# choice17/ransac_with_homography

Measured on AMD Instinct MI355X. Metric: backward-warp Mpixels/sec (+ RANSAC hypotheses/sec), higher is better.
Workload: dtype u8 (f64 coordinates, f32 blend); 1 GPU; transformImageH warp 3840x2160 RGB u8 bilinear -> 2028x3771 u8, 32 distinct frames per GPU per step, Hs mild perspective; full=False

## Files before the change

### ransac_with_homography_amd/csrc/rwh_warp_rgb8.h

```cpp
#pragma once
#include "rwh_common.h"
#include <type_traits>

namespace rwh {

typedef float f2 __attribute__((ext_vector_type(2)));

constexpr double MAGIC = 1572864.0;
constexpr uint32_t MAGIC_HI = 0x41380000u;
constexpr unsigned long long MAGIC_BITS = 0x4138000000000000ull;
constexpr float W_SCALE = 5.42101086242752217e-20f;
constexpr float U8_BIAS = -0.5f + 3.0517578125e-05f;

constexpr int FP_PX = 4;
constexpr int FP_ROWS = 9;
constexpr int FP_LANES = 21;
constexpr int FP_TEXELS = 4 * FP_LANES;
constexpr int FP_PITCH = 4 * FP_TEXELS + 16;

struct Coef {
    double cx[3], cy[3], cw[3];
    double dxs8[7][3];
    double ih[9];
    long long image;
// ... 838 lines not shown
            __builtin_amdgcn_wave_barrier();
            __builtin_amdgcn_fence(__ATOMIC_ACQUIRE, "wavefront");
        }
        const uint32_t bx = MAGIC_HI + (uint32_t)wxmn, by = MAGIC_HI + (uint32_t)wymn;
        const uint32_t rx_max = (uint32_t)(4 * wC - 2), ry_max = (uint32_t)(wnrows - 2);
#pragma unroll
        for (int h = 0; h < 2; ++h) {
            unsigned vbits = 0u;
            run_coords(h);
#pragma unroll
            for (int j = 0; j < FP_PX; ++j) {
                const bool valid = pixel_valid(j);
                weights2(lx[j], ly[j], valid ? WS : 0.f, valid ? WO : 0.f, valid ? WC : 0.f, wx0[j], wx1[j], wy0[j], wy1[j]);
                vbits |= (unsigned)valid << j;
                const uint32_t rx = min(hx[j] - bx, rx_max), ry = min(hy[j] - by, ry_max);
                const uint32_t lo = mad24_s(ry, (uint32_t)Win::LPITCH, rx << 2);
                const uint32_t* t0 = reinterpret_cast<const uint32_t*>(my + lo);
                const uint32_t* t1 = reinterpret_cast<const uint32_t*>(my + lo + Win::LPITCH);
                a0[j] = t0[0]; b0[j] = t0[1]; a1[j] = t1[0]; b1[j] = t1[1];
            }
            finish_masked_run(h, vbits);
        }
        return;
    }

    unsigned todo = 3u;
    if constexpr (HALVES) {
        todo = wpos ? 0u : 3u;
        if (wpos) {
            constexpr uint32_t lpitch = Win::LPITCH;
            chunk_t vh[2][Win::PASSES];
            int hrows[2];
            uint32_t tapc[2];
            bool hact[2];
#pragma unroll
            for (int h = 0; h < 2; ++h) {
                run_coords(h);
                const uint32_t lhx = h == 0 ? ehx[0] : hx[0], lhy = h == 0 ? ehy[0] : hy[0];
                const uint32_t rhx = h == 0 ? hx[3] : ehx[1], rhy = h == 0 ? hy[3] : ehy[1];
                const int hx0 = (int)__builtin_amdgcn_readlane(lhx, 0), hx1 = (int)__builtin_amdgcn_readlane(rhx, LPR - 1);
                const int hx2 = (int)__builtin_amdgcn_readlane(lhx, 64 - LPR), hx3 = (int)__builtin_amdgcn_readlane(rhx, 63);
                const int hy0 = (int)__builtin_amdgcn_readlane(lhy, 0), hy1 = (int)__builtin_amdgcn_readlane(rhy, LPR - 1);
                const int hy2 = (int)__builtin_amdgcn_readlane(lhy, 64 - LPR), hy3 = (int)__builtin_amdgcn_readlane(rhy, 63);
                const int qxmn = smin(smin(hx0, hx1), smin(hx2, hx3)) & ~3, qxmx = smax(smax(hx0, hx1), smax(hx2, hx3));
                const int qymn = smin(smin(hy0, hy1), smin(hy2, hy3)), qymx = smax(smax(hy0, hy1), smax(hy2, hy3));
                const int sxmn = (int)((uint32_t)smax(qxmn, 0) - MAGIC_HI), sxmx = (int)((uint32_t)smax(qxmx, 0) - MAGIC_HI);
                const int symn = (int)((uint32_t)smax(qymn, 0) - MAGIC_HI), symx = (int)((uint32_t)smax(qymx, 0) - MAGIC_HI);
                const int nr = symx - symn + 2, hC = (sxmx - sxmn + 5) >> 2;
                const bool hfits = (sxmn >= 0) & (sxmx < a.bound_w - 1) & (symn >= 0) & (symx < min(a.bound_h - 1, a.src_h - 2)) &
                                   (nr >= Win::RPP) & (nr <= Win::ROWS) & (hC <= Win::LPRW);
                hrows[h] = hfits ? nr : 0;
                hact[h] = (srow < Win::RPP) & (scol < hC);
                tapc[h] = ((uint32_t)qymn & 0xFFFFFFu) * lpitch + ((uint32_t)qxmn << 2) - slab_off_w;
                if (hfits) {
                    const unsigned char* gbase = simg + (size_t)((uint32_t)symn * pitch + (uint32_t)sxmn * (uint32_t)CH);
#pragma unroll
                    for (int p = 0; p < Win::PASSES; ++p)
                        if (p * Win::RPP < nr && hact[h])
                            __builtin_memcpy(&vh[h][p], gbase + (size_t)((uint32_t)min(p * Win::RPP, nr - Win::RPP) * pitch) + goff, sizeof(chunk_t));
                } else {
                    todo |= 1u << h;
                }
            }
#pragma unroll
            for (int h = 0; h < 2; ++h) {
                if (hrows[h] == 0) continue;
#pragma unroll
                for (int p = 0; p < Win::PASSES; ++p)
                    if (p * Win::RPP < hrows[h] && hact[h]) {
                        uint4 t4;
                        if constexpr (CH == 4) {
                            t4.x = vh[h][p].a; t4.y = vh[h][p].b; t4.z = vh[h][p].c; t4.w = vh[h][p].d;
                        } else {
                            t4.x = vh[h][p].a & 0xFFFFFFu;
                            t4.y = __builtin_amdgcn_perm(vh[h][p].b, vh[h][p].a, 0x0C050403u);
                            t4.z = __builtin_amdgcn_perm(vh[h][p].c, vh[h][p].b, 0x0C040302u);
                            t4.w = vh[h][p].c >> 8;
                        }
                        *reinterpret_cast<uint4*>(my + (uint32_t)min(p * Win::RPP, hrows[h] - Win::RPP) * lpitch + wl) = t4;
                    }
                __builtin_amdgcn_fence(__ATOMIC_RELEASE, "wavefront");
                __builtin_amdgcn_wave_barrier();
                __builtin_amdgcn_fence(__ATOMIC_ACQUIRE, "wavefront");
                if (h == 0) run_coords(0);
#pragma unroll
                for (int j = 0; j < FP_PX; ++j) {
                    weights2(lx[j], ly[j], WS, WO, WC, wx0[j], wx1[j], wy0[j], wy1[j]);
                    const uint32_t lo = mad24_s(hy[j], lpitch, shl2_add_s(hx[j], 0u - tapc[h]));
                    const uint32_t* t0 = reinterpret_cast<const uint32_t*>(slab0 + lo);
                    const uint32_t* t1 = reinterpret_cast<const uint32_t*>(slab0 + lo + lpitch);
                    a0[j] = t0[0]; b0[j] = t0[1]; a1[j] = t1[0]; b1[j] = t1[1];
                }
                const int first = tshift - (lcol + (PW / 2) * h);
                blend_store<DstT, PSTR, CH, true>(a0, b0, a1, b1, wx0, wx1, wy0, wy1, drow + CH * (PW / 2) * h,
                                                  store_any & (first <= 3 * PSTR), max(first, 0));
                __builtin_amdgcn_fence(__ATOMIC_RELEASE, "wavefront");
                __builtin_amdgcn_wave_barrier();
                if (h == 0 && hrows[1] != 0) run_coords(1);
            }
        }
        if (todo == 0u) return;
    }

#pragma unroll
    for (int h = 0; h < 2; ++h) {
        uint32_t off[FP_PX];
        bool near_end = false;
        unsigned vbits = 0u;
        if (HALVES && !(todo & (1u << h))) continue;
        run_coords(h);
#pragma unroll
        for (int j = 0; j < FP_PX; ++j) {
            const bool valid = pixel_valid(j);
            const int ix = (int)(hx[j] - MAGIC_HI), iy = (int)(hy[j] - MAGIC_HI);
            weights2(lx[j], ly[j], valid ? WS : 0.f, valid ? WO : 0.f, valid ? WC : 0.f, wx0[j], wx1[j], wy0[j], wy1[j]);
            off[j] = valid ? (uint32_t)iy * pitch + (uint32_t)ix * (uint32_t)CH : 0u;
            near_end |= valid & (iy > a.src_h - 3);
            vbits |= (unsigned)valid << j;
        }
        if (!__any(vbits != 0u)) {
#pragma unroll
            for (int j = 0; j < FP_PX; ++j) { a0[j] = 0u; b0[j] = 0u; a1[j] = 0u; b1[j] = 0u; }
        } else if (!__any(near_end)) {
#pragma unroll
            for (int j = 0; j < FP_PX; ++j) {
                const pk2 r0 = ld8(simg + off[j]);
                const pk2 r1 = ld8(simg + off[j] + pitch);
                if constexpr (CH == 4) { a0[j] = r0.a; b0[j] = r0.b; a1[j] = r1.a; b1[j] = r1.b; }
                else {
                    a0[j] = r0.a & 0xFFFFFFu; b0[j] = __builtin_amdgcn_perm(r0.b, r0.a, 0x0C050403u);
                    a1[j] = r1.a & 0xFFFFFFu; b1[j] = __builtin_amdgcn_perm(r1.b, r1.a, 0x0C050403u);
                }
            }
        } else {
            const uint32_t last = (uint32_t)a.src_h * pitch - (uint32_t)CH;
#pragma unroll
            for (int j = 0; j < FP_PX; ++j) {
                const uint32_t o00 = off[j];
                const uint32_t o01 = min(o00 + (uint32_t)CH, last), o10 = min(o00 + pitch, last), o11 = min(o00 + pitch + (uint32_t)CH, last);
                if constexpr (CH == 4) {
                    a0[j] = ld4(simg + o00); b0[j] = ld4(simg + o01); a1[j] = ld4(simg + o10); b1[j] = ld4(simg + o11);
                    continue;
                }
                a0[j] = simg[o00] | (simg[o00 + 1] << 8) | (simg[o00 + 2] << 16);
                b0[j] = simg[o01] | (simg[o01 + 1] << 8) | (simg[o01 + 2] << 16);
                a1[j] = simg[o10] | (simg[o10 + 1] << 8) | (simg[o10 + 2] << 16);
                b1[j] = simg[o11] | (simg[o11 + 1] << 8) | (simg[o11 + 2] << 16);
            }
        }
        finish_masked_run(h, vbits);
    }
}

constexpr int F8_WALK_WAVES = 4;
template <int LOG_PW> __device__ __forceinline__ void fast8mb_body(const FastArgs& a);
template <typename DstT, int LOG_PW, bool WALK = false>
__global__ __launch_bounds__(256, (WALK ? F8_WALK_WAVES : f8_waves<DstT, LOG_PW>())) void warp_rgb8_fast8(const FastArgs a) {
    if constexpr (WALK) {
        static_assert(sizeof(DstT) == 1, "the batch form is uint8 in, uint8 out");
        fast8mb_body<LOG_PW>(a);
    } else {
        fast8_body<DstT, LOG_PW>(a, nullptr);
    }
}
#ifndef RWH_F8H_WAVES
#define RWH_F8H_WAVES(log_pw) ((log_pw) == 5 ? 4 : 5)
#endif
template <int LOG_PW>
__global__ __launch_bounds__(256, RWH_F8H_WAVES(LOG_PW)) void warp_rgb8_fast8h(const FastArgs a) { fast8_body<unsigned char, LOG_PW, false, 3, true>(a, nullptr); }
template <int LOG_PW>
__global__ __launch_bounds__(256, RWH_F8H_WAVES(LOG_PW)) void warp_rgb8_fast8h_tab(const FastArgs a, const CoefTab t) { fast8_body<unsigned char, LOG_PW, false, 3, true>(a, t.e); }
template <int LOG_PW>
__global__ __launch_bounds__(256, 6) void warp_rgba8_fast8(const FastArgs a) { fast8_body<unsigned char, LOG_PW, false, 4>(a, nullptr); }
template <int LOG_PW>
__global__ __launch_bounds__(256, 6) void warp_rgb8_comp(const FastArgs a, const CompArgs c) { fast8_body<unsigned char, LOG_PW, true>(a, nullptr, &c); }
template <typename DstT, int LOG_PW>
__global__ __launch_bounds__(256, (f8_waves<DstT, LOG_PW>())) void warp_rgb8_fast8_tab(const FastArgs a, const CoefTab t) { fast8_body<DstT, LOG_PW>(a, t.e); }

__device__ __forceinline__ pk3 pack_run_u8(const float (&o)[FP_PX][3]) {
    pk3 w;
    uint32_t q = 0;
    q = __builtin_amdgcn_cvt_pk_u8_f32(o[0][0], 0, q); q = __builtin_amdgcn_cvt_pk_u8_f32(o[0][1], 1, q);
    q = __builtin_amdgcn_cvt_pk_u8_f32(o[0][2], 2, q); q = __builtin_amdgcn_cvt_pk_u8_f32(o[1][0], 3, q);
    w.a = q; q = 0;
    q = __builtin_amdgcn_cvt_pk_u8_f32(o[1][1], 0, q); q = __builtin_amdgcn_cvt_pk_u8_f32(o[1][2], 1, q);
    q = __builtin_amdgcn_cvt_pk_u8_f32(o[2][0], 2, q); q = __builtin_amdgcn_cvt_pk_u8_f32(o[2][1], 3, q);
    w.b = q; q = 0;
    q = __builtin_amdgcn_cvt_pk_u8_f32(o[2][2], 0, q); q = __builtin_amdgcn_cvt_pk_u8_f32(o[3][0], 1, q);
    q = __builtin_amdgcn_cvt_pk_u8_f32(o[3][1], 2, q); q = __builtin_amdgcn_cvt_pk_u8_f32(o[3][2], 3, q);
    w.c = q;
    return w;
}
__device__ __forceinline__ void store_run_pk(const pk3& w, unsigned char* drow, bool store_any, int shift) {
    if (!store_any) return;
#ifdef RWH_F8M_STORE_MOD
    if (shift == 0) {
        typedef uint32_t u3s __attribute__((ext_vector_type(3)));
        const u3s d = {w.a, w.b, w.c};
        asm volatile("global_store_dwordx3 %0, %1, off " RWH_F8M_STORE_MOD "\n\ts_nop 2" : : "v"(drow), "v"(d) : "memory");
        return;
    }
#else
    if (shift == 0) { __builtin_memcpy(drow, &w, 12); return; }
#endif
    const unsigned long long lo8 = ((unsigned long long)w.b << 32) | w.a;
#pragma unroll
    for (int i = 3; i < 12; ++i)
        if (i >= 3 * shift) drow[i] = (unsigned char)(i < 8 ? lo8 >> (8 * i) : w.c >> (8 * (i - 8)));
}
#ifndef RWH_F8M_SKEW
#define RWH_F8M_SKEW 8
#endif
__device__ __forceinline__ void store_run_u8(const float (&o)[FP_PX][3], unsigned char* drow, bool store_any, int shift) {
    if (!store_any) return;
    if (shift == 0) {
        pk3 w;
        uint32_t q = 0;
        q = __builtin_amdgcn_cvt_pk_u8_f32(o[0][0], 0, q); q = __builtin_amdgcn_cvt_pk_u8_f32(o[0][1], 1, q);
        q = __builtin_amdgcn_cvt_pk_u8_f32(o[0][2], 2, q); q = __builtin_amdgcn_cvt_pk_u8_f32(o[1][0], 3, q);
        w.a = q; q = 0;
        q = __builtin_amdgcn_cvt_pk_u8_f32(o[1][1], 0, q); q = __builtin_amdgcn_cvt_pk_u8_f32(o[1][2], 1, q);
        q = __builtin_amdgcn_cvt_pk_u8_f32(o[2][0], 2, q); q = __builtin_amdgcn_cvt_pk_u8_f32(o[2][1], 3, q);
        w.b = q; q = 0;
        q = __builtin_amdgcn_cvt_pk_u8_f32(o[2][2], 0, q); q = __builtin_amdgcn_cvt_pk_u8_f32(o[3][0], 1, q);
        q = __builtin_amdgcn_cvt_pk_u8_f32(o[3][1], 2, q); q = __builtin_amdgcn_cvt_pk_u8_f32(o[3][2], 3, q);
        w.c = q;
        __builtin_memcpy(drow, &w, 12);
    } else {
#pragma unroll
        for (int j = 1; j < FP_PX; ++j)
            if (j >= shift) {
#pragma unroll
                for (int k = 0; k < 3; ++k) drow[3 * j + k] = (unsigned char)__builtin_amdgcn_cvt_pk_u8_f32(o[j][k], 0, 0);
            }
    }
}

template <int LOG_PW>
__device__ __forceinline__ void fast8m_body(const FastArgs& a) {
    constexpr int PW = 1 << LOG_PW, PH = 512 / PW, LPR = PW / 8, WX = 128 / PW;
    using Win = F8Window<LOG_PW>;
    constexpr uint32_t lpitch = Win::LPITCH + RWH_F8M_SKEW;
    constexpr int SLAB = ((Win::ROWS * (int)lpitch + 15) / 16) * 16;
    static_assert(SLAB >= Win::SLAB, "the per-frame fallback body shares this slab");
    constexpr float WS = W_SCALE * MIX_S, WO = W_ONE * MIX_S, WC = MIX_S;
    static_assert(MIX_RGB, "the multi-frame kernel is written for the float16-halves blend");
    unsigned char* const slab0 = wave_slabs<SLAB>();

    const unsigned b = blockIdx.x;
    const unsigned logical = (b & 7u) * a.mf_cpx + (b >> 3);
    if (logical >= a.mf_nblocks) return;
    const unsigned g = a.ntiles_magic ? __umulhi(logical, a.ntiles_magic) : (a.ntiles == 1u ? logical : 0u);
    const unsigned ti = logical - g * a.ntiles;
    const int f0 = (int)g * a.mf_frames, f1 = min(f0 + a.mf_frames, a.mf_batch);
    const unsigned ty = a.tiles_x_magic ? __umulhi(ti, a.tiles_x_magic) : ti;
    const unsigned tx = ti - ty * a.tiles_x;
    const int wave = __builtin_amdgcn_readfirstlane((int)(threadIdx.x >> 6));
    const int pwave = wave;
    {
        const int own_from = (int)tx * 128 - min((int)tx * 128, a.out_w - 128);
        if ((wave % WX + 1) * PW <= own_from) return;
    }
    const Coef& co = a.c;
    const int lane = threadIdx.x & 63;
    const int prow = lane / LPR, pq = lane % LPR;
    const int wave_x = (wave % WX) * PW, wave_y = (wave / WX) * PH;
    const int rr_raw = (int)ty * 16 + wave_y + prow;
    const int rr = min(rr_raw, a.rows - 1);
    const int tcol0 = (int)tx * 128;
    const int tcol = min(tcol0, a.out_w - 128);
    const int tshift = tcol0 - tcol;
    const int lcol = wave_x + pq * 4;
    const int c0p = tcol + lcol;
    const bool store_any = rr_raw < a.rows;
    const uint32_t pitch = (uint32_t)a.src_w * 3u;

    const double fr = (double)(a.row_begin + rr), fc = (double)c0p;
    const double X0 = fma(fc, co.cx[2], fma(fr, co.cx[1], co.cx[0]));
    const double Y0 = fma(fc, co.cy[2], fma(fr, co.cy[1], co.cy[0]));
    const double W0 = fma(fc, co.cw[2], fma(fr, co.cw[1], co.cw[0]));
    uint32_t ehx[2], ehy[2], elx[2], ely[2];
    bool wpos;
    {
        const double X7 = X0 + co.dxs8[6][0], Y7 = Y0 + co.dxs8[6][1], W7 = W0 + co.dxs8[6][2];
        double r0 = __builtin_amdgcn_rcp(W0); r0 = fma(fma(-W0, r0, 1.0), r0, r0);
        double r7 = __builtin_amdgcn_rcp(W7); r7 = fma(fma(-W7, r7, 1.0), r7, r7);
        const double ux0 = fma(X0, r0, MAGIC), uy0 = fma(Y0, r0, MAGIC), ux7 = fma(X7, r7, MAGIC), uy7 = fma(Y7, r7, MAGIC);
        ehx[0] = hi32(ux0); elx[0] = lo32(ux0); ehy[0] = hi32(uy0); ely[0] = lo32(uy0);
        ehx[1] = hi32(ux7); elx[1] = lo32(ux7); ehy[1] = hi32(uy7); ely[1] = lo32(uy7);
        const int h0 = (int)hi32(W0), h7 = (int)hi32(W7);
        wpos = __all((int)(h0 > 0x2D300000) & (int)(h0 < 0x52B00000) & (int)(h7 > 0x2D300000) & (int)(h7 < 0x52B00000));
    }
    const int x0 = (int)__builtin_amdgcn_readlane(ehx[0], 0), x1 = (int)__builtin_amdgcn_readlane(ehx[1], LPR - 1);
    const int x2 = (int)__builtin_amdgcn_readlane(ehx[0], 64 - LPR), x3 = (int)__builtin_amdgcn_readlane(ehx[1], 63);
    const int y0 = (int)__builtin_amdgcn_readlane(ehy[0], 0), y1 = (int)__builtin_amdgcn_readlane(ehy[1], LPR - 1);
    const int y2 = (int)__builtin_amdgcn_readlane(ehy[0], 64 - LPR), y3 = (int)__builtin_amdgcn_readlane(ehy[1], 63);
    const int hxmn = smin(smin(x0, x1), smin(x2, x3)) & ~3, hxmx = smax(smax(x0, x1), smax(x2, x3));
    const int hymn = smin(smin(y0, y1), smin(y2, y3)), hymx = smax(smax(y0, y1), smax(y2, y3));
    const int xmn = (int)((uint32_t)smax(hxmn, 0) - MAGIC_HI), xmx = (int)((uint32_t)smax(hxmx, 0) - MAGIC_HI);
    const int ymn = (int)((uint32_t)smax(hymn, 0) - MAGIC_HI), ymx = (int)((uint32_t)smax(hymx, 0) - MAGIC_HI);
    const int nrows = ymx - ymn + 2, C = (xmx - xmn + 5) >> 2;
    const bool staged = wpos & (xmn >= 0) & (xmx < a.bound_w - 1) & (ymn >= 0) & (ymx < min(a.bound_h - 1, a.src_h - 2)) &
                        (nrows >= Win::RPP) & (nrows <= Win::ROWS) & (C <= Win::LPRW);
    if (!staged) {
        for (int f = f0; f < f1; ++f)
            fast8_body<unsigned char, LOG_PW, false, 3, false, true>(a, nullptr, nullptr, (int)((unsigned)f * a.ntiles + ti), slab0 + pwave * SLAB);
        return;
// ... 66 lines not shown
    float wa[F8_PX], wb[F8_PX], wc[F8_PX], wd[F8_PX];
    uint32_t lo[F8_PX];
#pragma unroll
    for (int h = 0; h < 2; ++h) {
        double X[3], Y[3], W[3], rc[3];
        uint32_t lx[FP_PX], ly[FP_PX], hx[FP_PX], hy[FP_PX];
#pragma unroll
        for (int j = 0; j < 3; ++j) { X[j] = X0 + co.dxs8[3 * h + j][0]; Y[j] = Y0 + co.dxs8[3 * h + j][1]; W[j] = W0 + co.dxs8[3 * h + j][2]; }
        const double p12 = W[0] * W[1], P = p12 * W[2];
        double rp = __builtin_amdgcn_rcp(P);
        rp = fma(fma(-P, rp, 1.0), rp, rp);
        const double r12 = rp * W[2];
        rc[2] = rp * p12; rc[0] = r12 * W[1]; rc[1] = r12 * W[0];
#pragma unroll
        for (int j = 0; j < 3; ++j) {
            const double ux = fma(X[j], rc[j], MAGIC), uy = fma(Y[j], rc[j], MAGIC);
            const int q = j + 1 - h;
            hx[q] = hi32(ux); lx[q] = lo32(ux); hy[q] = hi32(uy); ly[q] = lo32(uy);
        }
        hx[3 * h] = ehx[h]; lx[3 * h] = elx[h]; hy[3 * h] = ehy[h]; ly[3 * h] = ely[h];
#pragma unroll
        for (int j = 0; j < FP_PX; ++j) {
            const int p = 4 * h + j;
            const float wx1 = (float)lx[j], wy1 = (float)ly[j] * WS;
            const float w11 = wx1 * wy1;
            const float w01 = __builtin_fmaf(wx1, WO, -w11);
            const float w10 = __builtin_fmaf(wy1, 4294967296.0f, -w11);
            const float w00 = __builtin_fmaf(-wx1, WO, WC) - w10;
            wa[p] = w00; wb[p] = w01; wc[p] = w10; wd[p] = w11;
            lo[p] = mad24_s(hy[j], lpitch, shl2_add_s(hx[j], 0u - tap_c));
        }
    }

#ifdef RWH_F8M_EARLY1
#pragma unroll
    for (int p = 0; p < F8_PX; ++p) asm volatile("" : : "v"(wa[p]), "v"(wb[p]), "v"(wc[p]), "v"(wd[p]), "v"(lo[p]));
#else
    issue(gsrc, v1);
#endif
    landed(v1);
    expand(v1);
#ifndef RWH_F8M_EARLY2
    if (f0 + 1 < f1) issue(gsrc + a.src_img_stride, v);
#endif
#ifdef RWH_LAB_STAMPS
    unsigned long long tA = 0, tB = 0, tC = 0, tD = 0, t0 = __builtin_amdgcn_s_memtime(), t1;
#define RWH_STAMP(acc) { t1 = __builtin_amdgcn_s_memtime(); acc += t1 - t0; t0 = t1; }
#else
#define RWH_STAMP(acc)
#endif
    for (int f = f0; f < f1; ++f) {
        gsrc += a.src_img_stride;
        const bool more = f + 1 < f1;
        pk3 w[2];
#pragma unroll
        for (int h = 0; h < 2; ++h) {
            float o[FP_PX][3];
#pragma unroll
            for (int j = 0; j < FP_PX; ++j) {
                const int p = 4 * h + j;
                const uint32_t* t0 = reinterpret_cast<const uint32_t*>(slab0 + lo[p]);
                const uint32_t* t1 = reinterpret_cast<const uint32_t*>(slab0 + lo[p] + lpitch);
                const uint32_t a0 = t0[0], b0 = t0[1], a1 = t1[0], b1 = t1[1];
                const float w00 = wa[p], w01 = wb[p], w10 = wc[p], w11 = wd[p];
                const uint32_t g00 = rg_halves(a0), g01 = rg_halves(b0), g10 = rg_halves(a1), g11 = rg_halves(b1);
                o[j][0] = fmix_lo(g11, w11, fmix_lo(g10, w10, fmix_lo(g01, w01, fmix_lo_c(g00, w00, U8_BIAS))));
                o[j][1] = fmix_hi(g11, w11, fmix_hi(g10, w10, fmix_hi(g01, w01, fmix_hi_c(g00, w00, U8_BIAS))));
                o[j][2] = fmix_hi(b1, w11, fmix_hi(a1, w10, fmix_hi(b0, w01, fmix_hi_c(a0, w00, U8_BIAS))));
            }
            w[h] = pack_run_u8(o);
        }
        __builtin_amdgcn_fence(__ATOMIC_RELEASE, "wavefront");
        __builtin_amdgcn_wave_barrier();
        RWH_STAMP(tA)
        if (more) { landed(v); RWH_STAMP(tB) expand(v); }
        RWH_STAMP(tC)
        unsigned char* drow = gdst + doff;
#pragma unroll
        for (int h = 0; h < 2; ++h) {
            const int first = tshift - (lcol + (PW / 2) * h);
#ifdef RWH_ABL_M_NOSTORE
            if (w[h].a + w[h].b == 0x12345u)
#endif
            store_run_pk(w[h], drow + 3 * (PW / 2) * h, store_any & (first <= 3), max(first, 0));
        }
        gdst += a.dst_img_stride;
        if (f + 2 < f1) issue(gsrc + a.src_img_stride, v);
        RWH_STAMP(tD)
    }
#ifdef RWH_LAB_STAMPS
    if (lane == 0 && logical < 8192u) {
        unsigned long long* st = reinterpret_cast<unsigned long long*>(a.dst) + ((size_t)logical * 4 + pwave) * 4;
        st[0] = tA; st[1] = tB; st[2] = tC; st[3] = tD;
    }
#endif
}
constexpr int BCH = 36, BROWS = 22;
__device__ __forceinline__ void lds_barrier() { asm volatile("s_waitcnt lgkmcnt(0)\n\ts_barrier" : : : "memory"); }
template <int LOG_PW>
__device__ __forceinline__ void fast8mb_body(const FastArgs& a) {
    constexpr int PW = 1 << LOG_PW, PH = 512 / PW, LPR = PW / 8, WX = 128 / PW;
    using Win = F8Window<LOG_PW>;
    constexpr uint32_t lpitch = BCH * 16 + RWH_F8M_SKEW;
    constexpr int SLABW = ((Win::ROWS * (int)(Win::LPITCH + RWH_F8M_SKEW) + 15) / 16) * 16;
    static_assert(4 * SLABW >= BROWS * (int)lpitch + 128, "the block window lives in the four waves' slabs");
    constexpr float WS = W_SCALE * MIX_S, WO = W_ONE * MIX_S, WC = MIX_S;
    unsigned char* const slab0 = wave_slabs<SLABW>();

    const unsigned b = blockIdx.x;
    const unsigned logical = (b & 7u) * a.mf_cpx + (b >> 3);
    if (logical >= a.mf_nblocks) return;
    const unsigned g = a.ntiles_magic ? __umulhi(logical, a.ntiles_magic) : (a.ntiles == 1u ? logical : 0u);
    const unsigned ti = logical - g * a.ntiles;
    const int f0 = (int)g * a.mf_frames, f1 = min(f0 + a.mf_frames, a.mf_batch);
    const unsigned ty = a.tiles_x_magic ? __umulhi(ti, a.tiles_x_magic) : ti;
    const unsigned tx = ti - ty * a.tiles_x;
    const int wave = __builtin_amdgcn_readfirstlane((int)(threadIdx.x >> 6));
    const Coef& co = a.c;
    const int lane = threadIdx.x & 63;
    const int prow = lane / LPR, pq = lane % LPR;
    const int wave_x = (wave % WX) * PW, wave_y = (wave / WX) * PH;
    const int rr_raw = (int)ty * 16 + wave_y + prow;
    const int rr = min(rr_raw, a.rows - 1);
    const int tcol0 = (int)tx * 128;
    const int tcol = min(tcol0, a.out_w - 128);
    const int tshift = tcol0 - tcol;
    const int lcol = wave_x + pq * 4;
    const int c0p = tcol + lcol;
    const bool store_any = rr_raw < a.rows;
    const uint32_t pitch = (uint32_t)a.src_w * 3u;

    const double fr = (double)(a.row_begin + rr), fc = (double)c0p;
    const double X0 = fma(fc, co.cx[2], fma(fr, co.cx[1], co.cx[0]));
    const double Y0 = fma(fc, co.cy[2], fma(fr, co.cy[1], co.cy[0]));
    const double W0 = fma(fc, co.cw[2], fma(fr, co.cw[1], co.cw[0]));
    uint32_t ehx[2], ehy[2], elx[2], ely[2];
    bool wpos;
    {
        const double X7 = X0 + co.dxs8[6][0], Y7 = Y0 + co.dxs8[6][1], W7 = W0 + co.dxs8[6][2];
        double r0 = __builtin_amdgcn_rcp(W0); r0 = fma(fma(-W0, r0, 1.0), r0, r0);
        double r7 = __builtin_amdgcn_rcp(W7); r7 = fma(fma(-W7, r7, 1.0), r7, r7);
        const double ux0 = fma(X0, r0, MAGIC), uy0 = fma(Y0, r0, MAGIC), ux7 = fma(X7, r7, MAGIC), uy7 = fma(Y7, r7, MAGIC);
        ehx[0] = hi32(ux0); elx[0] = lo32(ux0); ehy[0] = hi32(uy0); ely[0] = lo32(uy0);
        ehx[1] = hi32(ux7); elx[1] = lo32(ux7); ehy[1] = hi32(uy7); ely[1] = lo32(uy7);
        const int h0 = (int)hi32(W0), h7 = (int)hi32(W7);
        wpos = __all((int)(h0 > 0x2D300000) & (int)(h0 < 0x52B00000) & (int)(h7 > 0x2D300000) & (int)(h7 < 0x52B00000));
    }
    const int x0 = (int)__builtin_amdgcn_readlane(ehx[0], 0), x1 = (int)__builtin_amdgcn_readlane(ehx[1], LPR - 1);
    const int x2 = (int)__builtin_amdgcn_readlane(ehx[0], 64 - LPR), x3 = (int)__builtin_amdgcn_readlane(ehx[1], 63);
    const int y0 = (int)__builtin_amdgcn_readlane(ehy[0], 0), y1 = (int)__builtin_amdgcn_readlane(ehy[1], LPR - 1);
    const int y2 = (int)__builtin_amdgcn_readlane(ehy[0], 64 - LPR), y3 = (int)__builtin_amdgcn_readlane(ehy[1], 63);
    const int whxmn = smin(smin(x0, x1), smin(x2, x3)) & ~3, whxmx = smax(smax(x0, x1), smax(x2, x3));
    const int whymn = smin(smin(y0, y1), smin(y2, y3)), whymx = smax(smax(y0, y1), smax(y2, y3));
    {
        const int xmn = (int)((uint32_t)smax(whxmn, 0) - MAGIC_HI), xmx = (int)((uint32_t)smax(whxmx, 0) - MAGIC_HI);
        const int ymn = (int)((uint32_t)smax(whymn, 0) - MAGIC_HI), ymx = (int)((uint32_t)smax(whymx, 0) - MAGIC_HI);
        const bool interior = wpos & (xmn >= 0) & (xmx < a.bound_w - 1) & (ymn >= 0) & (ymx < min(a.bound_h - 1, a.src_h - 2));
        int* red = reinterpret_cast<int*>(slab0);
        if (lane == 0) { red[5 * wave] = whxmn; red[5 * wave + 1] = whxmx; red[5 * wave + 2] = whymn; red[5 * wave + 3] = whymx; red[5 * wave + 4] = interior ? 1 : 0; }
    }
    __syncthreads();
    int hxmn, hxmx, hymn, hymx, all_in;
    {
        const int* red = reinterpret_cast<const int*>(slab0);
        hxmn = min(min(red[0], red[5]), min(red[10], red[15])); hxmx = max(max(red[1], red[6]), max(red[11], red[16]));
        hymn = min(min(red[2], red[7]), min(red[12], red[17])); hymx = max(max(red[3], red[8]), max(red[13], red[18]));
        all_in = red[4] & red[9] & red[14] & red[19];
        hxmn = __builtin_amdgcn_readfirstlane(hxmn); hxmx = __builtin_amdgcn_readfirstlane(hxmx);
        hymn = __builtin_amdgcn_readfirstlane(hymn); hymx = __builtin_amdgcn_readfirstlane(hymx);
        all_in = __builtin_amdgcn_readfirstlane(all_in);
    }
    __syncthreads();
    const int xmn = (int)((uint32_t)hxmn - MAGIC_HI), xmx = (int)((uint32_t)hxmx - MAGIC_HI);
    const int ymn = (int)((uint32_t)hymn - MAGIC_HI), ymx = (int)((uint32_t)hymx - MAGIC_HI);
    const int nrows = ymx - ymn + 2, C = (xmx - xmn + 5) >> 2;
    if (!(all_in && nrows <= BROWS && C <= BCH)) {
        const int own_from = (int)tx * 128 - min((int)tx * 128, a.out_w - 128);
        if ((wave % WX + 1) * PW <= own_from) return;
        for (int f = f0; f < f1; ++f)
            fast8_body<unsigned char, LOG_PW, false, 3, false, true>(a, nullptr, nullptr, (int)((unsigned)f * a.ntiles + ti), slab0 + wave * SLABW);
        return;
    }

    constexpr int SLOTS = (BROWS * BCH + 255) / 256;
    uint32_t goff[SLOTS], wl[SLOTS];
    unsigned long long smask[SLOTS];
    bool sact[SLOTS];
#pragma unroll
    for (int p = 0; p < SLOTS; ++p) {
        const int c = (int)threadIdx.x + 256 * p, r = c / BCH, k = c - r * BCH;
        sact[p] = (r < nrows) & (k < C);
        goff[p] = mad24_s((uint32_t)r, pitch, mul24_12((uint32_t)k));
        wl[p] = (uint32_t)r * lpitch + (uint32_t)k * 16u;
        smask[p] = __ballot(sact[p]);
    }
    const unsigned char* gsrc = a.src + (long long)f0 * a.src_img_stride + (size_t)((uint32_t)ymn * pitch + (uint32_t)xmn * 3u);
    unsigned char* gdst = a.dst + (long long)f0 * a.dst_img_stride;
    const uint32_t doff = ((uint32_t)rr * (uint32_t)a.pitch_w + (uint32_t)c0p) * 3u;
    typedef uint32_t u3 __attribute__((ext_vector_type(3)));
    auto issue = [&](const unsigned char* gb, u3 (&v)[SLOTS]) __attribute__((always_inline)) {
#pragma unroll
        for (int p = 0; p < SLOTS; ++p) {
            unsigned long long keep;
            asm volatile("s_mov_b64 %1, exec\n\ts_mov_b64 exec, %4\n\tglobal_load_dwordx3 %0, %2, %3\n\ts_mov_b64 exec, %1"
                         : "=&v"(v[p]), "=&s"(keep) : "v"(goff[p]), "s"(gb), "s"(smask[p]) : "memory");
        }
    };
    auto landed = [&](u3 (&v)[SLOTS]) __attribute__((always_inline)) {
        static_assert(SLOTS == 4, "operand list below");
        asm volatile("s_waitcnt vmcnt(0)" : "+v"(v[0]), "+v"(v[1]), "+v"(v[2]), "+v"(v[3]) : : "memory");
    };
    auto expand = [&](const u3 (&v)[SLOTS]) __attribute__((always_inline)) {
#pragma unroll
        for (int p = 0; p < SLOTS; ++p)
            if (sact[p]) {
                uint4 t4;
                t4.x = v[p].x & 0xFFFFFFu;
                t4.y = __builtin_amdgcn_perm(v[p].y, v[p].x, 0x0C050403u);
                t4.z = __builtin_amdgcn_perm(v[p].z, v[p].y, 0x0C040302u);
                t4.w = v[p].z >> 8;
                __builtin_memcpy(__builtin_assume_aligned(slab0 + wl[p], RWH_F8M_SKEW % 16 ? 8 : 16), &t4, 16);
            }
    };

    const uint32_t tap_c = ((uint32_t)hymn & 0xFFFFFFu) * lpitch + ((uint32_t)hxmn << 2);
    float wa[F8_PX], wb[F8_PX], wc[F8_PX], wd[F8_PX];
    uint32_t lo[F8_PX];
#pragma unroll
    for (int h = 0; h < 2; ++h) {
        double X[3], Y[3], W[3], rc[3];
        uint32_t lx[FP_PX], ly[FP_PX], hx[FP_PX], hy[FP_PX];
#pragma unroll
        for (int j = 0; j < 3; ++j) { X[j] = X0 + co.dxs8[3 * h + j][0]; Y[j] = Y0 + co.dxs8[3 * h + j][1]; W[j] = W0 + co.dxs8[3 * h + j][2]; }
        const double p12 = W[0] * W[1], P = p12 * W[2];
        double rp = __builtin_amdgcn_rcp(P);
        rp = fma(fma(-P, rp, 1.0), rp, rp);
        const double r12 = rp * W[2];
        rc[2] = rp * p12; rc[0] = r12 * W[1]; rc[1] = r12 * W[0];
#pragma unroll
        for (int j = 0; j < 3; ++j) {
            const double ux = fma(X[j], rc[j], MAGIC), uy = fma(Y[j], rc[j], MAGIC);
            const int q = j + 1 - h;
            hx[q] = hi32(ux); lx[q] = lo32(ux); hy[q] = hi32(uy); ly[q] = lo32(uy);
        }
        hx[3 * h] = ehx[h]; lx[3 * h] = elx[h]; hy[3 * h] = ehy[h]; ly[3 * h] = ely[h];
#pragma unroll
        for (int j = 0; j < FP_PX; ++j) {
            const int p = 4 * h + j;
            const float wx1 = (float)lx[j], wy1 = (float)ly[j] * WS;
            const float w11 = wx1 * wy1;
            const float w01 = __builtin_fmaf(wx1, WO, -w11);
            const float w10 = __builtin_fmaf(wy1, 4294967296.0f, -w11);
            const float w00 = __builtin_fmaf(-wx1, WO, WC) - w10;
            wa[p] = w00; wb[p] = w01; wc[p] = w10; wd[p] = w11;
            lo[p] = mad24_s(hy[j], lpitch, shl2_add_s(hx[j], 0u - tap_c));
        }
    }
    u3 v[SLOTS];
    issue(gsrc, v);
    landed(v);
    expand(v);
    lds_barrier();
    if (f0 + 1 < f1) issue(gsrc + a.src_img_stride, v);
    for (int f = f0; f < f1; ++f) {
        gsrc += a.src_img_stride;
        const bool more = f + 1 < f1;
        pk3 w[2];
#pragma unroll
        for (int h = 0; h < 2; ++h) {
            float o[FP_PX][3];
#pragma unroll
            for (int j = 0; j < FP_PX; ++j) {
                const int p = 4 * h + j;
                const uint32_t* t0 = reinterpret_cast<const uint32_t*>(slab0 + lo[p]);
                const uint32_t* t1 = reinterpret_cast<const uint32_t*>(slab0 + lo[p] + lpitch);
                const uint32_t a0 = t0[0], b0 = t0[1], a1 = t1[0], b1 = t1[1];
                const float w00 = wa[p], w01 = wb[p], w10 = wc[p], w11 = wd[p];
                const uint32_t g00 = rg_halves(a0), g01 = rg_halves(b0), g10 = rg_halves(a1), g11 = rg_halves(b1);
                o[j][0] = fmix_lo(g11, w11, fmix_lo(g10, w10, fmix_lo(g01, w01, fmix_lo_c(g00, w00, U8_BIAS))));
                o[j][1] = fmix_hi(g11, w11, fmix_hi(g10, w10, fmix_hi(g01, w01, fmix_hi_c(g00, w00, U8_BIAS))));
                o[j][2] = fmix_hi(b1, w11, fmix_hi(a1, w10, fmix_hi(b0, w01, fmix_hi_c(a0, w00, U8_BIAS))));
            }
            w[h] = pack_run_u8(o);
        }
        if (more) {
            lds_barrier();
            landed(v);
            expand(v);
            lds_barrier();
        }
        unsigned char* drow = gdst + doff;
#pragma unroll
        for (int h = 0; h < 2; ++h) {
            const int first = tshift - (lcol + (PW / 2) * h);
            store_run_pk(w[h], drow + 3 * (PW / 2) * h, store_any & (first <= 3), max(first, 0));
        }
        gdst += a.dst_img_stride;
        if (f + 2 < f1) issue(gsrc + a.src_img_stride, v);
    }
}
template <int LOG_PW>
__global__ __launch_bounds__(256, 4) void warp_rgb8_fast8mb(const FastArgs a) { fast8mb_body<LOG_PW>(a); }

#ifndef RWH_F8M_WAVES
#define RWH_F8M_WAVES 4
#endif
template <int LOG_PW>
__global__ __launch_bounds__(256, RWH_F8M_WAVES) void warp_rgb8_fast8m(const FastArgs a) { fast8m_body<LOG_PW>(a); }

#ifndef RWH_STRIP_MAX
#define RWH_STRIP_MAX 16
#endif
constexpr int STRIP_MAX = RWH_STRIP_MAX;
template <typename DstT>
__device__ __forceinline__ void strip_body(const FastArgs& a, const Coef* tab) {
    constexpr bool U8 = sizeof(DstT) == 1;
    constexpr float WS = W_SCALE * MIX_S, WO = W_ONE * MIX_S, WC = MIX_S, BIAS = U8 ? U8_BIAS : 0.f;
    const int rr = (int)(blockIdx.x * 256 + threadIdx.x);
    const unsigned img = blockIdx.y;
    if (rr >= a.rows) return;
    const Coef& co = tab ? tab[img] : a.c;
    const unsigned img_mem = tab ? (unsigned)co.image : img;
    const unsigned char* simg = a.src + (long long)img_mem * a.src_img_stride;
    DstT* drow = reinterpret_cast<DstT*>(a.dst + (long long)img_mem * a.dst_img_stride) + ((size_t)rr * (size_t)a.pitch_w) * 3;
    const uint32_t pitch = (uint32_t)a.src_w * 3u, last = (uint32_t)a.src_h * pitch - 3u;
    const double fr = (double)(a.row_begin + rr);
    for (int c = a.out_w; c < a.pitch_w; ++c) {
        const double fc = (double)c;
        const double X = fma(fc, co.cx[2], fma(fr, co.cx[1], co.cx[0]));
        const double Y = fma(fc, co.cy[2], fma(fr, co.cy[1], co.cy[0]));
        const double W = fma(fc, co.cw[2], fma(fr, co.cw[1], co.cw[0]));
        double r = __builtin_amdgcn_rcp(W);
        r = fma(fma(-W, r, 1.0), r, r);
        const double ux = fma(X, r, MAGIC), uy = fma(Y, r, MAGIC);
        const unsigned long long ubx = (unsigned long long)__double_as_longlong(ux), uby = (unsigned long long)__double_as_longlong(uy);
        const bool valid = (ubx >= MAGIC_BITS) & (ubx <= a.xmax_bits) & (uby >= MAGIC_BITS) & (uby <= a.ymax_bits);
        float o[3] = {BIAS, BIAS, BIAS};
        if (valid) {
            const int ix = (int)(hi32(ux) - MAGIC_HI), iy = (int)(hi32(uy) - MAGIC_HI);
            const float wx1 = (float)lo32(ux), wy1 = (float)lo32(uy) * WS;
            const float w11 = wx1 * wy1;
            const float w01 = __builtin_fmaf(wx1, WO, -w11);
            const float w10 = __builtin_fmaf(wy1, 4294967296.0f, -w11);
            const float w00 = __builtin_fmaf(-wx1, WO, WC) - w10;
            const uint32_t o00 = (uint32_t)iy * pitch + (uint32_t)ix * 3u;
            const uint32_t o01 = min(o00 + 3u, last), o10 = min(o00 + pitch, last), o11 = min(o00 + pitch + 3u, last);
#pragma unroll
            for (int k = 0; k < 3; ++k) {
                const float p00 = (float)simg[o00 + k] * 0x1p-24f, p01 = (float)simg[o01 + k] * 0x1p-24f;
                const float p10 = (float)simg[o10 + k] * 0x1p-24f, p11 = (float)simg[o11 + k] * 0x1p-24f;
                o[k] = __builtin_fmaf(p11, w11, __builtin_fmaf(p10, w10, __builtin_fmaf(p01, w01, __builtin_fmaf(p00, w00, BIAS))));
            }
        }
#pragma unroll
        for (int k = 0; k < 3; ++k) {
            if constexpr (U8) drow[3 * c + k] = (unsigned char)__builtin_amdgcn_cvt_pk_u8_f32(o[k], 0, 0);
            else drow[3 * c + k] = o[k];
        }
    }
}
template <typename DstT>
__global__ __launch_bounds__(256) void warp_rgb8_strip(const FastArgs a) { strip_body<DstT>(a, nullptr); }
template <typename DstT>
__global__ __launch_bounds__(256) void warp_rgb8_strip_tab(const FastArgs a, const CoefTab t) { strip_body<DstT>(a, t.e); }

constexpr uint32_t NN_TIE = 1u << 12;

__device__ __forceinline__ uint32_t nn_exact_texel(const FastArgs& a, const double (&ih)[9], const unsigned char* simg, int r, int c) {
    const double x = (c == a.out_w - 1) ? a.gx_last : (double)c * a.gstep_x + a.gx0;
    const double y = (r == a.out_h - 1) ? a.gy_last : (double)r * a.gstep_y + a.gy0;
    const double X = fma(ih[1], y, ih[0] * x) + ih[2];
    const double Y = fma(ih[4], y, ih[3] * x) + ih[5];
    const double W = fma(ih[7], y, ih[6] * x) + ih[8];
    const double sx = X / W, sy = Y / W;
    const int xi = (int)(sx + 0.5), yi = (int)(sy + 0.5);
    if (!((xi >= 0) & (xi <= a.bound_w - 1) & (yi >= 0) & (yi <= a.bound_h - 1) & (sx == sx) & (sy == sy))) return 0u;
    const uint32_t off = ((uint32_t)yi * (uint32_t)a.src_w + (uint32_t)xi) * 3u;
    const uint32_t img_bytes = (uint32_t)a.src_h * (uint32_t)a.src_w * 3u;
    if (off + 4u <= img_bytes) return ld4(simg + off) & 0xFFFFFFu;
    return simg[off] | (simg[off + 1] << 8) | (simg[off + 2] << 16);
}

__device__ __forceinline__ void nn_store(const uint32_t (&t)[FP_PX], unsigned char* drow, bool store_any, int first) {
    if (!store_any) return;
    if (first <= 0) {
        pk3 w;
        w.a = (t[0] & 0xFFFFFFu) | (t[1] << 24);
        w.b = ((t[1] >> 8) & 0xFFFFu) | (t[2] << 16);
        w.c = ((t[2] >> 16) & 0xFFu) | (t[3] << 8);
        __builtin_memcpy(drow, &w, 12);
    } else {
#pragma unroll
        for (int j = 1; j < FP_PX; ++j)
            if (j >= first) { drow[3 * j] = (unsigned char)t[j]; drow[3 * j + 1] = (unsigned char)(t[j] >> 8); drow[3 * j + 2] = (unsigned char)(t[j] >> 16); }
    }
}

template <int LOG_PW>
__device__ __forceinline__ void nn_body(const FastArgs& a, const Coef* tab) {
    constexpr int PW = 1 << LOG_PW, PH = 512 / PW, LPR = PW / 8, WX = 128 / PW;
    constexpr double MAGIC_R = MAGIC + 0.5;
    __shared__ __attribute__((aligned(16))) unsigned char slab[4][F8Window<LOG_PW>::SLAB];

    const unsigned b = blockIdx.x;
    const unsigned logical = (b & 7u) * a.cpx + (b >> 3);
    if (logical >= a.nblocks) return;
    const unsigned t = a.tiles_x_magic ? __umulhi(logical, a.tiles_x_magic) : logical;
    const unsigned tx = logical - t * a.tiles_x;
    const unsigned img = a.tiles_y_magic ? __umulhi(t, a.tiles_y_magic) : t;
    const unsigned ty = t - img * a.tiles_y;
    const Coef& co = tab ? tab[img] : a.c;
    const unsigned img_mem = tab ? (unsigned)co.image : img;
    double ih9[9];
#pragma unroll
    for (int i = 0; i < 9; ++i) ih9[i] = co.ih[i];
    const int wave = __builtin_amdgcn_readfirstlane((int)(threadIdx.x >> 6));
    const int lane = threadIdx.x & 63;
    const int prow = lane / LPR, pq = lane % LPR;
    const int wave_x = (wave % WX) * PW, wave_y = (wave / WX) * PH;
    const int rr_raw = (int)ty * 16 + wave_y + prow;
    const int rr = min(rr_raw, a.rows - 1);
    const int tcol0 = (int)tx * 128, tcol = min(tcol0, a.out_w - 128), tshift = tcol0 - tcol;
    if ((wave_x + PW <= tshift) | ((int)ty * 16 + wave_y >= a.rows)) return;
    const int lcol = wave_x + pq * 4, c0p = tcol + lcol;
    const bool store_any = rr_raw < a.rows;
    const unsigned char* simg = a.src + (long long)img_mem * a.src_img_stride;
    unsigned char* drow = a.dst + (long long)img_mem * a.dst_img_stride + ((uint32_t)rr * (uint32_t)a.pitch_w + (uint32_t)c0p) * 3u;
    const uint32_t pitch = (uint32_t)a.src_w * 3u;
    const int out_row = a.row_begin + rr;

    const double fr = (double)out_row, fc = (double)c0p;
    const double X0 = fma(fc, co.cx[2], fma(fr, co.cx[1], co.cx[0]));
    const double Y0 = fma(fc, co.cy[2], fma(fr, co.cy[1], co.cy[0]));
    const double W0 = fma(fc, co.cw[2], fma(fr, co.cw[1], co.cw[0]));
    uint32_t ehx[2], ehy[2], elx[2], ely[2];
    bool wpos;
    {
        const double X7 = X0 + co.dxs8[6][0], Y7 = Y0 + co.dxs8[6][1], W7 = W0 + co.dxs8[6][2];
        double r0 = __builtin_amdgcn_rcp(W0); r0 = fma(fma(-W0, r0, 1.0), r0, r0);
        double r7 = __builtin_amdgcn_rcp(W7); r7 = fma(fma(-W7, r7, 1.0), r7, r7);
        const double ux0 = fma(X0, r0, MAGIC_R), uy0 = fma(Y0, r0, MAGIC_R), ux7 = fma(X7, r7, MAGIC_R), uy7 = fma(Y7, r7, MAGIC_R);
        ehx[0] = hi32(ux0); elx[0] = lo32(ux0); ehy[0] = hi32(uy0); ely[0] = lo32(uy0);
        ehx[1] = hi32(ux7); elx[1] = lo32(ux7); ehy[1] = hi32(uy7); ely[1] = lo32(uy7);
        const int h0 = (int)hi32(W0), h7 = (int)hi32(W7);
        wpos = __all((int)(h0 > 0x2D300000) & (int)(h0 < 0x52B00000) & (int)(h7 > 0x2D300000) & (int)(h7 < 0x52B00000));
    }
    uint32_t lx[FP_PX], ly[FP_PX], hx[FP_PX], hy[FP_PX];
    auto run_coords = [&](const int h) {
// ... 139 lines not shown
```

Measured before the change: 691,800 Mpix/s.

## Extend multi-frame LDS staging path to edge tiles with masked taps and zero-fill

The multi-frame batched warp kernel now handles border blocks instead of falling back to the per-frame slow path. Block bounds are clamped to the source and computed only from waves that actually overlap the source. Per-pixel validity masking zeroes the weights and clamps tap offsets into the staged slab. Blocks entirely outside the source just zero-store, and waves that are fully outside skip the compute. The occupancy hint for the walk kernel is also raised from 4 to 5 waves, which adds register pressure and more branching.

```diff
diff --git a/ransac_with_homography_amd/csrc/rwh_warp_rgb8.h b/ransac_with_homography_amd/csrc/rwh_warp_rgb8.h
--- a/ransac_with_homography_amd/csrc/rwh_warp_rgb8.h
+++ b/ransac_with_homography_amd/csrc/rwh_warp_rgb8.h
@@ -1014,7 +1014,7 @@
     }
 }
 
-constexpr int F8_WALK_WAVES = 4;
+constexpr int F8_WALK_WAVES = 5;
 template <int LOG_PW> __device__ __forceinline__ void fast8mb_body(const FastArgs& a);
 template <typename DstT, int LOG_PW, bool WALK = false>
 __global__ __launch_bounds__(256, (WALK ? F8_WALK_WAVES : f8_waves<DstT, LOG_PW>())) void warp_rgb8_fast8(const FastArgs a) {
@@ -1387,33 +1387,55 @@
     const int y2 = (int)__builtin_amdgcn_readlane(ehy[0], 64 - LPR), y3 = (int)__builtin_amdgcn_readlane(ehy[1], 63);
     const int whxmn = smin(smin(x0, x1), smin(x2, x3)) & ~3, whxmx = smax(smax(x0, x1), smax(x2, x3));
     const int whymn = smin(smin(y0, y1), smin(y2, y3)), whymx = smax(smax(y0, y1), smax(y2, y3));
+    const bool owns = (wave % WX + 1) * PW > tshift;
+    bool in;
     {
-        const int xmn = (int)((uint32_t)smax(whxmn, 0) - MAGIC_HI), xmx = (int)((uint32_t)smax(whxmx, 0) - MAGIC_HI);
-        const int ymn = (int)((uint32_t)smax(whymn, 0) - MAGIC_HI), ymx = (int)((uint32_t)smax(whymx, 0) - MAGIC_HI);
-        const bool interior = wpos & (xmn >= 0) & (xmx < a.bound_w - 1) & (ymn >= 0) & (ymx < min(a.bound_h - 1, a.src_h - 2));
+        const int bxmn = (int)((uint32_t)smax(whxmn, 0) - MAGIC_HI), bxmx = (int)((uint32_t)smax(whxmx, 0) - MAGIC_HI);
+        const int bymn = (int)((uint32_t)smax(whymn, 0) - MAGIC_HI), bymx = (int)((uint32_t)smax(whymx, 0) - MAGIC_HI);
+        const bool outside = wpos & ((bxmx < 0) | (bxmn >= a.bound_w) | (bymx < 0) | (bymn >= a.bound_h));
+        const bool interior = wpos & (bxmn >= 0) & (bxmx < a.bound_w - 1) & (bymn >= 0) & (bymx < min(a.bound_h - 1, a.src_h - 2));
+        in = owns & !outside;
+        const int bw1 = __builtin_amdgcn_readfirstlane(a.bound_w) - 1, bh1 = __builtin_amdgcn_readfirstlane(a.bound_h) - 1;
         int* red = reinterpret_cast<int*>(slab0);
-        if (lane == 0) { red[5 * wave] = whxmn; red[5 * wave + 1] = whxmx; red[5 * wave + 2] = whymn; red[5 * wave + 3] = whymx; red[5 * wave + 4] = interior ? 1 : 0; }
+        if (lane == 0) {
+            red[5 * wave] = in ? smin(smax(bxmn, 0), bw1) : 0x7FFFFFFF; red[5 * wave + 1] = in ? smin(smax(bxmx, 0), bw1) : -0x7FFFFFFF - 1;
+            red[5 * wave + 2] = in ? smin(smax(bymn, 0), bh1) : 0x7FFFFFFF; red[5 * wave + 3] = in ? smin(smax(bymx, 0), bh1) : -0x7FFFFFFF - 1;
+            red[5 * wave + 4] = (wpos ? 1 : 0) | ((interior | !owns) ? 2 : 0);
+        }
     }
     __syncthreads();
-    int hxmn, hxmx, hymn, hymx, all_in;
+    int xmn, xmx, ymn, ymx, fl_and;
     {
         const int* red = reinterpret_cast<const int*>(slab0);
-        hxmn = min(min(red[0], red[5]), min(red[10], red[15])); hxmx = max(max(red[1], red[6]), max(red[11], red[16]));
-        hymn = min(min(red[2], red[7]), min(red[12], red[17])); hymx = max(max(red[3], red[8]), max(red[13], red[18]));
-        all_in = red[4] & red[9] & red[14] & red[19];
-        hxmn = __builtin_amdgcn_readfirstlane(hxmn); hxmx = __builtin_amdgcn_readfirstlane(hxmx);
-        hymn = __builtin_amdgcn_readfirstlane(hymn); hymx = __builtin_amdgcn_readfirstlane(hymx);
-        all_in = __builtin_amdgcn_readfirstlane(all_in);
+        xmn = min(min(red[0], red[5]), min(red[10], red[15])); xmx = max(max(red[1], red[6]), max(red[11], red[16]));
+        ymn = min(min(red[2], red[7]), min(red[12], red[17])); ymx = max(max(red[3], red[8]), max(red[13], red[18]));
+        fl_and = red[4] & red[9] & red[14] & red[19];
+        xmn = __builtin_amdgcn_readfirstlane(xmn) & ~3; xmx = __builtin_amdgcn_readfirstlane(xmx);
+        ymn = __builtin_amdgcn_readfirstlane(ymn); ymx = __builtin_amdgcn_readfirstlane(ymx);
+        fl_and = __builtin_amdgcn_readfirstlane(fl_and);
     }
     __syncthreads();
-    const int xmn = (int)((uint32_t)hxmn - MAGIC_HI), xmx = (int)((uint32_t)hxmx - MAGIC_HI);
-    const int ymn = (int)((uint32_t)hymn - MAGIC_HI), ymx = (int)((uint32_t)hymx - MAGIC_HI);
-    const int nrows = ymx - ymn + 2, C = (xmx - xmn + 5) >> 2;
-    if (!(all_in && nrows <= BROWS && C <= BCH)) {
-        const int own_from = (int)tx * 128 - min((int)tx * 128, a.out_w - 128);
-        if ((wave % WX + 1) * PW <= own_from) return;
+    const bool any_in = ymn != 0x7FFFFFFF;
+    const int nrows = any_in ? ymx - ymn + 2 : 0, C = any_in ? (xmx - xmn + 5) >> 2 : 0;
+    const uint32_t doff = ((uint32_t)rr * (uint32_t)a.pitch_w + (uint32_t)c0p) * 3u;
+    const bool masked = !(fl_and & 2);
+    if (!(fl_and & 1) || (any_in && !(nrows <= BROWS && C <= BCH && ymn + nrows - 1 <= a.src_h - 2))) {
+        if (!owns) return;
         for (int f = f0; f < f1; ++f)
             fast8_body<unsigned char, LOG_PW, false, 3, false, true>(a, nullptr, nullptr, (int)((unsigned)f * a.ntiles + ti), slab0 + wave * SLABW);
+        return;
+    }
+    if (!any_in) {
+        if (!owns) return;
+        unsigned char* drow = a.dst + (long long)f0 * a.dst_img_stride + doff;
+        for (int f = f0; f < f1; ++f) {
+#pragma unroll
+            for (int h = 0; h < 2; ++h) {
+                const int first = tshift - (lcol + (PW / 2) * h);
+                zero_store<unsigned char, 1, 3>(drow + 3 * (PW / 2) * h, store_any & (first <= 3), max(first, 0));
+            }
+            drow += a.dst_img_stride;
+        }
         return;
     }
 
@@ -1431,7 +1453,6 @@
     }
     const unsigned char* gsrc = a.src + (long long)f0 * a.src_img_stride + (size_t)((uint32_t)ymn * pitch + (uint32_t)xmn * 3u);
     unsigned char* gdst = a.dst + (long long)f0 * a.dst_img_stride;
-    const uint32_t doff = ((uint32_t)rr * (uint32_t)a.pitch_w + (uint32_t)c0p) * 3u;
     typedef uint32_t u3 __attribute__((ext_vector_type(3)));
     auto issue = [&](const unsigned char* gb, u3 (&v)[SLOTS]) __attribute__((always_inline)) {
 #pragma unroll
@@ -1458,9 +1479,12 @@
             }
     };
 
-    const uint32_t tap_c = ((uint32_t)hymn & 0xFFFFFFu) * lpitch + ((uint32_t)hxmn << 2);
+    const uint32_t bx = MAGIC_HI + (uint32_t)xmn, by = MAGIC_HI + (uint32_t)ymn;
+    const uint32_t rx_max = (uint32_t)(4 * C - 2), ry_max = (uint32_t)(nrows - 2);
+    const uint32_t tap_c = (by & 0xFFFFFFu) * lpitch + (bx << 2);
     float wa[F8_PX], wb[F8_PX], wc[F8_PX], wd[F8_PX];
     uint32_t lo[F8_PX];
+    if (in) {
 #pragma unroll
     for (int h = 0; h < 2; ++h) {
         double X[3], Y[3], W[3], rc[3];
@@ -1479,17 +1503,36 @@
             hx[q] = hi32(ux); lx[q] = lo32(ux); hy[q] = hi32(uy); ly[q] = lo32(uy);
         }
         hx[3 * h] = ehx[h]; lx[3 * h] = elx[h]; hy[3 * h] = ehy[h]; ly[3 * h] = ely[h];
-#pragma unroll
-        for (int j = 0; j < FP_PX; ++j) {
-            const int p = 4 * h + j;
-            const float wx1 = (float)lx[j], wy1 = (float)ly[j] * WS;
-            const float w11 = wx1 * wy1;
-            const float w01 = __builtin_fmaf(wx1, WO, -w11);
-            const float w10 = __builtin_fmaf(wy1, 4294967296.0f, -w11);
-            const float w00 = __builtin_fmaf(-wx1, WO, WC) - w10;
-            wa[p] = w00; wb[p] = w01; wc[p] = w10; wd[p] = w11;
-            lo[p] = mad24_s(hy[j], lpitch, shl2_add_s(hx[j], 0u - tap_c));
-        }
+        if (!masked) {
+#pragma unroll
+            for (int j = 0; j < FP_PX; ++j) {
+                const int p = 4 * h + j;
+                const float wx1 = (float)lx[j], wy1 = (float)ly[j] * WS;
+                const float w11 = wx1 * wy1;
+                const float w01 = __builtin_fmaf(wx1, WO, -w11);
+                const float w10 = __builtin_fmaf(wy1, 4294967296.0f, -w11);
+                const float w00 = __builtin_fmaf(-wx1, WO, WC) - w10;
+                wa[p] = w00; wb[p] = w01; wc[p] = w10; wd[p] = w11;
+                lo[p] = mad24_s(hy[j], lpitch, shl2_add_s(hx[j], 0u - tap_c));
+            }
+        } else {
+#pragma unroll
+            for (int j = 0; j < FP_PX; ++j) {
+                const int p = 4 * h + j;
+                const unsigned long long ubx = ((unsigned long long)hx[j] << 32) | lx[j], uby = ((unsigned long long)hy[j] << 32) | ly[j];
+                const bool valid = (ubx >= MAGIC_BITS) & (ubx <= a.xmax_bits) & (uby >= MAGIC_BITS) & (uby <= a.ymax_bits);
+                const float ws = valid ? WS : 0.f, wo = valid ? WO : 0.f, wc1 = valid ? WC : 0.f;
+                const float wx1 = (float)lx[j], wy1 = (float)ly[j] * ws;
+                const float w11 = wx1 * wy1;
+                const float w01 = __builtin_fmaf(wx1, wo, -w11);
+                const float w10 = __builtin_fmaf(wy1, 4294967296.0f, -w11);
+                const float w00 = __builtin_fmaf(-wx1, wo, wc1) - w10;
+                wa[p] = w00; wb[p] = w01; wc[p] = w10; wd[p] = w11;
+                const uint32_t rx = min(hx[j] - bx, rx_max), ry = min(hy[j] - by, ry_max);
+                lo[p] = mad24_s(ry, lpitch, rx << 2);
+            }
+        }
+    }
     }
     u3 v[SLOTS];
     issue(gsrc, v);
@@ -1501,6 +1544,7 @@
         gsrc += a.src_img_stride;
         const bool more = f + 1 < f1;
         pk3 w[2];
+        if (in) {
 #pragma unroll
         for (int h = 0; h < 2; ++h) {
             float o[FP_PX][3];
@@ -1518,6 +1562,7 @@
             }
             w[h] = pack_run_u8(o);
         }
+        }
         if (more) {
             lds_barrier();
             landed(v);
@@ -1525,10 +1570,18 @@
             lds_barrier();
         }
         unsigned char* drow = gdst + doff;
-#pragma unroll
-        for (int h = 0; h < 2; ++h) {
-            const int first = tshift - (lcol + (PW / 2) * h);
-            store_run_pk(w[h], drow + 3 * (PW / 2) * h, store_any & (first <= 3), max(first, 0));
+        if (in) {
+#pragma unroll
+            for (int h = 0; h < 2; ++h) {
+                const int first = tshift - (lcol + (PW / 2) * h);
+                store_run_pk(w[h], drow + 3 * (PW / 2) * h, store_any & (first <= 3), max(first, 0));
+            }
+        } else if (owns) {
+#pragma unroll
+            for (int h = 0; h < 2; ++h) {
+                const int first = tshift - (lcol + (PW / 2) * h);
+                zero_store<unsigned char, 1, 3>(drow + 3 * (PW / 2) * h, store_any & (first <= 3), max(first, 0));
+            }
         }
         gdst += a.dst_img_stride;
         if (f + 2 < f1) issue(gsrc + a.src_img_stride, v);
```

Result: faster. 713,400 Mpix/s (median of 6 runs) (+3.1%).
